# weidafeng/Efficient-SlowFast

Hardware: AMD Instinct MI355X
Metric: clips/sec (8x8 224^2 SlowFast-R50+CMDA, train step fwd+bwd+allreduce+SGD) (higher is better)
Workload: dtype f32

## Files before the change

efficient-slowfast_amd/sfhip/__init__.py:

```python
import ctypes
import os

import torch

_HERE = os.path.dirname(os.path.abspath(__file__))
_LIB_PATH = os.environ.get("SF_LIB") or os.path.join(_HERE, "libsfhip.so")
_lib = None

ACT_NONE, ACT_RELU, ACT_SIGMOID, ACT_SOFTMAX, ACT_HSIGMOID, ACT_RELU6 = 0, 1, 2, 3, 4, 5


def _act(relu):
    return ACT_RELU6 if relu == 6 else (ACT_RELU if relu else ACT_NONE)
SF_EINVAL, SF_EALIGN, SF_ELAUNCH, SF_ENOTTAKEN = -1, -2, -3, -4
_ERR = {-1: "SF_EINVAL (inconsistent descriptor)", -2: "SF_EALIGN", -3: "SF_ELAUNCH (hip launch failed)",
        -4: "SF_ENOTTAKEN (shape not served by this specialised entry point)"}
_REFUSED = (SF_EALIGN, SF_ENOTTAKEN)


class SfhipError(RuntimeError):
    pass


class ConvDesc(ctypes.Structure):
# ... 80 lines not shown
    "sf_attn_fwd_ws_floats": (_cl, [_ci] * 3),
    "sf_attn_products_per_fp32": (_ci, [_ci]),
    "sf_attn_fwd_ws": (_ci, _ATTN_FWD + [_vp, _vp]),
    "sf_attn_bwd": (_ci, [_vp, _ci] * 4 + [_vp, _vp, _vp] + [_vp, _ci] * 3 + [_ci] * 4 + [_vp]),
    "sf_attn_bwd_fused_ws_floats": (_cl, [_ci] * 3),
    "sf_attn_bwd_fused": (_ci, [_vp, _ci] * 4 + [_vp, _vp, _vp] + [_vp, _ci] * 3 + [_ci] * 3 + [_vp, _vp]),
    "sf_attn_bwd_variant": (_ci, [_ci] * 3),
    "sf_attn_tune": (_ci, [_ci, _ci]),
    "sf_xattn_accepts": (_ci, [_cl, _cl, _ci, _ci]),
    "sf_xattn_bwd_ws_floats": (_cl, [_ci, _cl, _cl, _ci, _ci]),
    "sf_xattn_fwd": (_ci, [_vp, _ci] * 4 + [_vp, _ci, _cl, _cl, _ci, _ci, _cf, _vp]),
    "sf_xattn_bwd": (_ci, [_vp, _ci] * 4 + [_vp, _vp] + [_vp, _ci] * 3 + [_ci, _ci, _cl, _cl, _ci, _ci, _cf, _vp, _vp]),
    "sf_assoc_accepts": (_ci, [_cl, _cl, _ci, _ci]),
    "sf_gram_splits": (_ci, [_ci, _cl, _ci, _ci]),
    "sf_gram_ws_floats": (_cl, [_ci, _cl, _ci, _ci]),
    "sf_gram": (_ci, [_vp, _ci, _vp, _ci, _vp, _vp, _ci, _cl, _ci, _ci, _cf, _vp, _vp]),
    "sf_rowmat": (_ci, [_vp, _ci, _vp, _vp, _ci, _ci, _cl, _ci, _ci, _cf, _ci, _vp]),
    "sf_channel_stats_ws_floats": (_cl, [_ci]),
    "sf_channel_stats": (_ci, _VIEW + [_cl, _ci, _vp, _vp, _vp, _vp]),
    "sf_bn_train_stats": (_ci, _VIEW + [_cl, _ci, _vp, _vp, _cf, _cf] + [_vp] * 9),
    "sf_bn_train_stats_split": (_ci, _VIEW + [_ci, _cl, _ci, _ci, _vp, _vp, _cf, _cf] + [_vp] * 9),
    "sf_bn_train_stats_merge": (_ci, [_vp, _ci, _ci, _vp, _vp, _cf, _cf] + [_vp] * 8),
    "sf_affine_fwd": (_ci, _VIEW + [_ci] * 5 + [_vp, _vp] + _VIEW + [_ci, _ci] + _VIEW + [_ci, _vp]),
    "sf_affine_fwd_split": (_ci, _VIEW + [_ci] * 6 + [_vp, _vp] + _VIEW + [_ci, _ci] + _VIEW + [_ci, _vp]),
    "sf_affine_fwd_mask": (_ci, _VIEW + [_ci] * 5 + [_vp, _vp] + _VIEW + [_ci] + _VIEW + [_vp, _vp]),
    "sf_bn_bwd_ws_floats": (_cl, [_ci]),
    "sf_bn_bwd_reduce": (_ci, _BN_BWD + [_vp]),
    "sf_bn_bwd_reduce_acc": (_ci, _BN_BWD + [_vp, _vp, _vp]),
    "sf_bn_bwd_reduce_split": (_ci, _BN_BWD_SPLIT + [_vp]),
    "sf_bn_bwd_apply": (_ci, _BN_BWD + _BN_APPLY_TAIL),
    "sf_bn_bwd_apply_first": (_ci, _BN_BWD + _BN_APPLY_TAIL),
    "sf_bn_bwd_apply_split": (_ci, _BN_BWD_SPLIT + _BN_APPLY_TAIL),
    "sf_bn_frozen_bwd": (_ci, _VIEW * 3 + [_ci] * 7 + [_vp] * 3 + _VIEW * 2 + [_ci] + [_vp] * 4),
    "sf_head_act_mean": (_ci, [_vp, _ci, _ci, _ci, _ci, _vp, _vp]),
    "sf_head_act_mean_bwd": (_ci, [_vp, _vp, _ci, _ci, _ci, _ci, _vp, _ci, _vp]),
    "sf_copy_channels": (_ci, _VIEW * 2 + [_ci, _cl, _ci, _vp]),
    "sf_channel_shuffle": (_ci, _VIEW * 2 + [_ci, _cl, _ci, _ci, _vp]),
    "sf_gather_add": (_ci, _VIEW + [_ci] + _VIEW + [_cl, _ci, _ci, _vp]),
    "sf_bcast_add": (_ci, _VIEW + [_ci, _cl, _ci, _vp, _cf, _vp]),
    "sf_rowdot": (_ci, _VIEW * 2 + [_cl, _ci, _cf, _vp, _vp]),
    "sf_axpy": (_ci, _VIEW + [_cf] + _VIEW + [_cl, _ci, _ci, _vp]),
    "sf_act_bwd": (_ci, _VIEW * 2 + [_ci] + _VIEW + [_cl, _ci, _ci, _vp]),
    "sf_sigmoid_bwd": (_ci, [_vp, _vp, _vp, _cl, _ci, _vp]),
    "sf_row_softmax_fwd": (_ci, _VIEW + [_cl, _ci, _cf, _vp]),
    "sf_row_softmax_bwd": (_ci, _VIEW * 2 + [_cl, _ci, _cf, _vp]),
    "sf_roi_tpool_fwd": (_ci, _VIEW + [_ci] * 5 + [_vp, _vp]),
    "sf_roi_align_max_fwd": (_ci, [_vp] + [_ci] * 4 + [_vp, _ci, _ci, _cf, _ci] + _VIEW + [_vp, _vp]),
    "sf_roi_align_max_bwd": (_ci, _VIEW + [_vp, _vp] + [_ci] * 7 + [_cf, _ci] + _VIEW + [_ci, _vp]),
    "sf_epilogue_bwd": (_ci, _VIEW * 2 + [_ci] * 6 + [_vp, _ci] + _VIEW + [_ci] + _VIEW + [_ci, _vp]),
    "sf_epilogue_bwd_act": (_ci, _VIEW * 2 + [_ci] * 6 + [_vp, _ci, _ci] + _VIEW + [_ci] + _VIEW + [_ci, _vp]),
    "sf_cam_weights": (_ci, _VIEW + [_ci] * 5 + [_vp, _vp]),
    "sf_cam_map_ws_floats": (_cl, [_ci] * 4),
    "sf_cam_map": (_ci, _VIEW + [_vp] + [_ci] * 5 + [_vp, _vp, _vp, _vp]),
    "sf_ctx_pool_parts": (_ci, [_cl]),
    "sf_ctx_pool_ws_floats": (_cl, [_ci, _cl, _ci]),
    "sf_ctx_pool_fwd": (_ci, _VIEW + [_ci, _cl, _ci] + [_vp] * 6),
    "sf_ctx_pool_bwd": (_ci, _VIEW + [_ci, _cl, _ci] + [_vp] * 5 + _VIEW + [_ci, _vp, _vp, _ci, _vp, _vp]),
    "sf_sample_affine_ws_floats": (_cl, [_ci, _cl, _ci]),
    "sf_sample_affine_fwd": (_ci, _VIEW + [_ci, _cl, _ci, _vp, _vp] + _VIEW + [_vp]),
    "sf_sample_affine_bwd": (_ci, _VIEW * 2 + [_ci, _cl, _ci, _vp] + _VIEW + [_ci, _vp, _vp, _vp, _vp]),
    "sf_stripe_pool_fwd": (_ci, _VIEW + [_ci] * 7 + _VIEW + [_vp, _vp]),
    "sf_stripe_add_fwd": (_ci, _VIEW * 2 + [_ci] * 6 + _VIEW + [_vp]),
    "sf_stripe_pool_bwd": (_ci, _VIEW * 3 + [_vp] + [_ci] * 6 + _VIEW + [_ci, _vp]),
}
EXPORTS = list(_SIGNATURES)

# ... 811 lines not shown
    _call("sf_conv_fwd_grouped", ctypes.byref(d), groups, 0, dz.ptr(), _ptr(wtp), None, None,
          out.ptr() if accumulate else None, out.ptr(), tag=("conv", dz.rows, taps * (dz.C // groups), cin),
          what="sf_conv_fwd_grouped(transposed)")
    return out


def conv_wgrad_grouped(x, dz, groups, kernel, stride=(1, 1, 1), padding=(0, 0, 0), dilation=(1, 1, 1),
                       cin_pad=None, finish_into=None):
    _require_gpu(x.buf, "conv_wgrad_grouped")
    cin_g, cout = x.C // groups, dz.C
    assert x.C % groups == 0 and cout % groups == 0
    cin_pad = _pad16(cin_g) if cin_pad is None else cin_pad
    kT, kH, kW = kernel
    d = _conv_desc(x, (dz.T, dz.H, dz.W), 0, 0, cout, kernel, stride, padding, dilation, cin_pad=cin_pad)
    S = lib().sf_conv_wgrad_grouped_splits(ctypes.byref(d), groups)
    if S <= 0:
        raise SfhipError("sf_conv_wgrad_grouped_splits: %d -> %d channels in %d groups" % (x.C, cout, groups))
    part = torch.empty((S, cout, kT * kH * kW, cin_pad), dtype=torch.float32, device=x.buf.device)
    _call("sf_conv_wgrad_grouped", ctypes.byref(d), groups, x.ptr(), dz.ptr(), dz.cs, dz.coff, _ptr(part),
          tag=("conv", dz.rows, kT * kH * kW * cin_g, cout))
    if finish_into is not None:
        dst = finish_into
        assert dst.is_contiguous() and dst.dtype == torch.float32 and dst.numel() == cout * cin_g * kT * kH * kW
        _call("sf_conv_wgrad_finish", _ptr(part), S, cout, kT * kH * kW, cin_pad, cin_g, 0, _ptr(dst), 1)
        return None
    return part.sum(0) if S > 1 else part[0]


def unpack_conv_weight_grad(dwp, shape):
    cout, cin, kT, kH, kW = shape
    return dwp[:, :, :cin].permute(0, 2, 1).reshape(cout, cin, kT, kH, kW).contiguous()


def bn_bwd(dy, y, z, mean, invstd, gamma, relu, rep=1, dres=None, dz_out=None, dgamma_out=None, nsplit=1,
           sync=None, grad_sink=None, mask=None, dres_overwrite=False):
    C = z.C
    dev = z.buf.device
    mean, invstd, gamma = mean.contiguous(), invstd.contiguous(), gamma.detach().contiguous()
    dbeta = torch.empty((nsplit * C,), dtype=torch.float32, device=dev)
    dgamma = torch.empty((nsplit * C,), dtype=torch.float32, device=dev)
    ws = torch.empty((lib().sf_bn_bwd_ws_floats(C),), dtype=torch.float32, device=dev)
    yp, ycs, yco = (y.ptr(), y.cs, y.coff) if y is not None else (None, 0, 0)
    code = 2 if relu == 6 else (1 if relu else 0)
    if mask is not None and relu:
        assert rep == 1 and nsplit == 1 and mask.numel() == z.rows * (C // 4)
        yp, ycs, yco, code = _ptr(mask), C // 4, 0, 3
    head = (dy.ptr(), dy.cs, dy.coff, yp, ycs, yco, z.ptr(), z.cs, z.coff, z.N, z.T, z.H, z.W, C)
    tail = (rep, code, _ptr(mean), _ptr(invstd))
    split = (nsplit,) if nsplit > 1 else ()
    reduce_fn = "sf_bn_bwd_reduce_split" if nsplit > 1 else "sf_bn_bwd_reduce"
    apply_fn = "sf_bn_bwd_apply_split" if nsplit > 1 else "sf_bn_bwd_apply"
    if dres_overwrite:
        assert dres is not None and nsplit == 1
        apply_fn = "sf_bn_bwd_apply_first"
    if grad_sink is not None:
        assert nsplit == 1 and dgamma_out is None
        _call("sf_bn_bwd_reduce_acc", *head, *tail, _ptr(dbeta), _ptr(dgamma), _ptr(ws), _ptr(grad_sink[1]),
              _ptr(grad_sink[0]))
    else:
        _call(reduce_fn, *head, *split, *tail, _ptr(dbeta), _ptr(dgamma), _ptr(ws))
    db_apply, dg_apply = (dbeta, dgamma) if sync is None else sync(dbeta, dgamma)
    out = z if dz_out is None else dz_out
    _call(apply_fn, *head, *split, *tail, _ptr(gamma), _ptr(db_apply), _ptr(dg_apply), out.ptr(), out.cs, out.coff,
          dres.ptr() if dres is not None else None, dres.cs if dres is not None else 0,
          dres.coff if dres is not None else 0)
    if dgamma_out is not None:
        if nsplit > 1:
            dgamma_out[0][:C] = dgamma.view(nsplit, C).sum(0)
            dgamma_out[1][:C] = dbeta.view(nsplit, C).sum(0)
        else:
            dgamma_out[0][:C] = dgamma
            dgamma_out[1][:C] = dbeta
    return out, dgamma, dbeta


def bn_frozen_bwd(dy, y, z, mean, invstd, gamma, relu, rep=1, dres=None, dres_overwrite=False, dz_out=None,
                  grads=None, mask=None):
    if dy is None or z is None or (relu and mask is None and y is None):
        raise SfhipError("bn_frozen_bwd: dy, z and (with an activation) y or its mask are required")
    for name, a in (("dy", dy), ("z", z), ("dz", dz_out), ("dres", dres), ("y", y if (relu and mask is None) else None)):
        if a is not None:
            _require_gpu(a.buf, "bn_frozen_bwd(%s)" % name)
    C, dev = z.C, z.buf.device
    if dres is not None and rep != 1:
        raise SfhipError("bn_frozen_bwd: the residual's gradient is only defined without a T repeat (rep = %d)" % rep)
    if (dy.N, dy.T, dy.H, dy.W, dy.C) != (z.N, z.T * rep, z.H, z.W, C):
        raise SfhipError("bn_frozen_bwd: dy %r does not match z %r repeated %d times" % (dy, z, rep))
    vecs = [("mean", mean), ("invstd", invstd)] + ([("gamma", gamma)] if gamma is not None else [])
    for name, v in vecs:
        _require_gpu(v, "bn_frozen_bwd(%s)" % name)
        if v.numel() < C or not v.is_contiguous():
            raise SfhipError("bn_frozen_bwd: %s must be a contiguous tensor of at least %d floats" % (name, C))
    dgp = dbp = ws = None
    if grads is not None:
        for name, v in (("dgamma", grads[0]), ("dbeta", grads[1])):
            _require_gpu(v, "bn_frozen_bwd(%s)" % name)
            if v.numel() < C or not v.is_contiguous():
                raise SfhipError("bn_frozen_bwd: %s must be a contiguous tensor of at least %d floats" % (name, C))
# ... 556 lines not shown
```

efficient-slowfast_amd/slowfast/models/engine.py:

```python
import os
import threading
import weakref

import torch
import torch.nn as nn

import sfhip
from sfhip import Act

_tls = threading.local()


class internal(object):

    def __enter__(self):
        self.prev = getattr(_tls, "depth", 0)
        _tls.depth = self.prev + 1

    def __exit__(self, *a):
        _tls.depth = self.prev


def is_internal():
    return getattr(_tls, "depth", 0) > 0
# ... 263 lines not shown
        _tls.pending_side = None
    else:
        _tls.pending_side = side
    if t is not None:
        t.record(bwd_fork)
    return [out0, out1]


def join_pending(device):
    pend = getattr(_tls, "pending_side", None)
    if pend is not None:
        _sync_streams(pend, torch.cuda.current_stream(device))
        _tls.pending_side = None


class taping(object):
    def __init__(self, t):
        self.t = t

    def __enter__(self):
        self.prev = getattr(_tls, "tape", None)
        _tls.tape = self.t

    def __exit__(self, *a):
        _tls.tape = self.prev


def _colsum(act):
    mean, _ = sfhip.channel_stats(act)
    return mean * float(act.rows)


def _record_conv(x, conv_weight, conv_bias, wp_shape, gsrc, kernel, stride, padding, dilation, x_needs_grad=True,
                 cin=None, unpack=None, fold_kw=0):
    t = tape()
    if t is None:
        return
    cout = conv_weight.shape[0]

    def wgrad(g):
        tgt = t.pgrad_target(conv_weight)
        if tgt is not None:
            real_cin = conv_weight.shape[1]
            sfhip.conv_wgrad(x, g, cout, kernel, stride, padding, dilation, cin=cin, cin_pad=wp_shape[2],
                             finish_into=(tgt, real_cin, fold_kw))
        else:
            dwp = sfhip.conv_wgrad(x, g, cout, kernel, stride, padding, dilation, cin=cin, cin_pad=wp_shape[2])
            t.add_pgrad(conv_weight, unpack(dwp) if unpack else sfhip.unpack_conv_weight_grad(dwp, conv_weight.shape))
        if conv_bias is not None:
            t.add_pgrad(conv_bias, _colsum(g))

    def bwd():
        g = gsrc() if callable(gsrc) else gsrc
        dev = x.buf.device
        if not t.param_grads:
            pass
        elif OVERLAP_PATHS and not t.capturing and not t.serial and x_needs_grad and dev.type == "cuda":
            cur = torch.cuda.current_stream(dev)
            wg = _companion_stream(cur)
            _sync_streams(cur, wg)
            with torch.cuda.stream(wg):
                wgrad(g)
            g.buf.record_stream(wg)
            x.buf.record_stream(wg)
            t.joins.add(wg)
        else:
            wgrad(g)
        if x_needs_grad:
            if conv_weight.dim() == 5 and tuple(conv_weight.shape[2:]) == tuple(kernel):
                wtp = _packed_pair(conv_weight)[1]
            else:
                wtp = _cached_t(conv_weight, "_sf_wtp", _key(conv_weight),
                                lambda: sfhip.pack_conv_weight(conv_weight.detach().reshape(
                                    conv_weight.shape[0], conv_weight.shape[1], *kernel).transpose(0, 1).contiguous()))
            fresh = t.grad_of_uninitialised(x)
            if fresh is not None:
                sfhip.conv_dgrad(g, wtp, x, kernel, stride, padding, dilation, out=fresh, accumulate=False)
            else:
                sfhip.conv_dgrad(g, wtp, x, kernel, stride, padding, dilation, out=t.grad_of(x), accumulate=True)

    t.record(bwd)


_PCACHE = {}


_CAPTURE_KEEP = {}


def _keep_if_capturing(obj):
    if getattr(_tls, "capturing", False):
        _CAPTURE_KEEP[id(obj)] = obj
    return obj


def _cached_t(tensor, slot, key, make):
    store = tensor.__dict__.setdefault("_sf_cache", {})
    c = store.get(slot)
    if c is None or c[0] != key:
        with torch.no_grad():
            c = (key, make())
        store[slot] = c
    return _keep_if_capturing(c[1])


_PARAM_EPOCH = 0


def parameters_changed(*_unused):
    global _PARAM_EPOCH
    _PARAM_EPOCH += 1


def replay(graph):
# ... 77 lines not shown
        vec = group_gather_sum(torch.cat([lm, lvar.double() + lm * lm]), nd, ng) / nd
        mean64, meansqr = vec[:z.C], vec[z.C:]
        var64 = (meansqr - mean64 * mean64).clamp_min(0.0)
        mean, var = mean64.float(), var64.float()
        invstd = torch.rsqrt(var64 + bn.eps).float()
        scale = (bn.weight.detach() * invstd).contiguous()
        shift = (bn.bias.detach() - mean * scale).contiguous()
        if track:
            bn.running_mean += m * (mean - bn.running_mean)
            bn.running_var += m * (var - bn.running_var)
            bn.__dict__.pop("_sf_affine", None)

        def sync(dbeta, dgamma):
            tot = group_gather_sum(torch.cat([dbeta, dgamma]).double(), nd, ng) / nd
            return tot[:dbeta.numel()].float().contiguous(), tot[dbeta.numel():].float().contiguous()

        return mean, invstd, scale, shift, 1, bn.weight, sync
    if conv_stats is not None:
        mean, invstd, scale, shift = sfhip.bn_train_stats_merge(
            conv_stats, z.C, bn.weight, bn.bias, bn.eps, m, bn.running_mean if track else None,
            bn.running_var if track else None)
    else:
        mean, invstd, scale, shift = sfhip.bn_train_stats(
            z, bn.weight, bn.bias, bn.eps, m, bn.running_mean if track else None, bn.running_var if track else None)
    if track:
        bn.__dict__.pop("_sf_affine", None)
        _bump(bn.num_batches_tracked)
    return mean, invstd, scale, shift, 1, bn.weight, None


def bn_train_apply(bn, z, res=None, relu=False, rep=1, out=None, out_reserve=(0, 0), keep=None, out_cmul=1,
                   conv_stats=None):
    check_bn(bn)
    with torch.no_grad():
        mean, invstd, scale, shift, nsplit, gamma_b, sync = _bn_train_stats(bn, z, conv_stats)
    zz = z if keep is None else z.slice(0, keep)
    nk = z.C if keep is None else keep
    if keep is not None:
        assert nsplit == 1, "channel-sliced BN (GhostModule) is only defined for plain BatchNorm3d"
        scale, shift = scale[:keep].contiguous(), shift[:keep].contiguous()
    t = tape()
    shuffled = t is not None and out_cmul != 1
    mk = {} if (t is not None and relu) else None
    if shuffled:
        y = sfhip.affine(zz, scale.contiguous(), shift.contiguous(), res=res, relu=relu, rep=rep, nsplit=nsplit,
                         mask=mk)
    else:
        y = sfhip.affine(zz, scale.contiguous(), shift.contiguous(), res=res, relu=relu, rep=rep, out=out,
                         out_reserve=out_reserve, out_cmul=out_cmul, nsplit=nsplit, mask=mk)
    mask = mk.get("bytes") if mk else None
    if t is not None:
        if _GRAD_SINK:
            dg = db = None
        else:
            dg = torch.zeros(z.C, dtype=torch.float32, device=z.buf.device)
            db = torch.zeros(z.C, dtype=torch.float32, device=z.buf.device)
        sel = slice(None) if nsplit > 1 else slice(0, nk)

        def bwd():
            dres, first = None, False
            if res is not None:
                fresh = t.grad_of_uninitialised(res) if (nsplit == 1 and res.C == zz.C and rep == 1) else None
                dres, first = (fresh, True) if fresh is not None else (t.grad_of(res), False)
            wt = t.pgrad_target(bn.weight) if (nsplit == 1 and getattr(bn, "weight", None) is not None) else None
            bt = t.pgrad_target(bn.bias) if wt is not None else None
            if wt is not None and bt is not None:
                sfhip.bn_bwd(t.grad_of(y), y, zz, mean[sel], invstd[sel], gamma_b[sel], relu, rep=rep, dres=dres,
                             dz_out=zz, sync=sync, grad_sink=(wt, bt), mask=mask, dres_overwrite=first)
            else:
                dg_ = dg if dg is not None else torch.zeros(z.C, dtype=torch.float32, device=z.buf.device)
                db_ = db if db is not None else torch.zeros(z.C, dtype=torch.float32, device=z.buf.device)
                sfhip.bn_bwd(t.grad_of(y), y, zz, mean[sel], invstd[sel], gamma_b[sel], relu, rep=rep, dres=dres,
                             dz_out=zz, dgamma_out=(dg_, db_), nsplit=nsplit, sync=sync, mask=mask,
                             dres_overwrite=first)
            if keep is not None and keep < z.C:
                rest = z.slice(keep, z.C - keep)
                sfhip.axpy(rest, rest, alpha=0.0, accumulate=False)
            if (wt is None or bt is None) and getattr(bn, "weight", None) is not None:
                t.add_pgrad(bn.weight, dg_)
                t.add_pgrad(bn.bias, db_)

        t.record(bwd)
    if shuffled:
        return copy_channels(y, out, out_cmul=out_cmul)
    return y


def bn_affine(bn, conv_bias=None):
    check_bn(bn)
    stat = bn.bn if _sub_bn(bn) else bn
    w = getattr(bn, "weight", None)
    b = getattr(bn, "bias", None)

    def make():
        inv = 1.0 / torch.sqrt(stat.running_var + stat.eps)
        scale = w * inv if w is not None else inv
        bias = -stat.running_mean * scale
        if b is not None:
            bias = bias + b
        if conv_bias is not None:
            bias = bias + scale * conv_bias
        return scale.detach().contiguous(), bias.detach().contiguous()

    return _cached(bn, "_sf_affine", _key(w, b, stat.running_mean, stat.running_var, conv_bias), make)


def _taped_training():
# ... 194 lines not shown
    if t is not None:
        t.record(lambda: sfhip.channel_shuffle(t.grad_of(out), t.grad_of(x), x.C // groups, accumulate=True))
    return out


def _is_grouped(conv):
    return 1 < conv.groups and not (conv.groups == conv.in_channels and conv.out_channels == conv.in_channels)


def conv_bn_act(x, conv, bn=None, relu=False, res=None, out=None, out_reserve=(0, 0), out_cmul=1, cout=None,
                shuffle=False):
    if _is_grouped(conv):
        assert out_cmul == 1 and cout is None, "grouped convs have their own shuffle"
        if bn is not None and bn_unfused(bn):
            z = grouped_conv(x, conv, bias=conv.bias)
            _record_grouped_conv(x, conv, z)
            if not shuffle:
                return bn_apply(bn, z, res=res, relu=relu, out=out, out_reserve=out_reserve)
            y = bn_apply(bn, z, res=res, relu=relu)
            return channel_shuffle(y, conv.groups, out=out, out_reserve=out_reserve)
        scale, bias = bn_affine(bn, conv.bias) if bn is not None else (None, conv.bias)
        t = tape()
        if t is not None and not isinstance(t, EvalTape):
            raise NotImplementedError("taped grouped conv without a norm layer behind it")
        y = grouped_conv(x, conv, scale=scale, bias=bias, relu=relu, res=res, out=out, out_reserve=out_reserve,
                         shuffle=shuffle)
        if t is not None:
            _record_eval_grouped_conv(t, x, conv, y, scale, relu, res, shuffle)
        return y
    assert not shuffle or conv.groups == 1, "channel_shuffle of a depthwise conv's output is not used by any model"
    wp = packed_weight(conv)
    if bn is not None and bn_unfused(bn):
        k, s, p, d = conv.kernel_size, conv.stride, conv.padding, conv.dilation
        st = None
        if conv.groups == 1:
            want = bn.training and _plain_bn(bn) and bn.affine
            z = sfhip.conv(x, wp, k, s, p, d, bias=conv.bias, stats=want)
            z, st = z if want else (z, None)
            _record_conv(x, conv.weight, conv.bias, wp.shape, z, k, s, p, d)
        else:
            ones = _cached(conv, "_sf_ones", (conv.out_channels, str(x.buf.device)),
                           lambda: torch.ones(conv.out_channels, dtype=torch.float32, device=x.buf.device))
            z = sfhip.dwconv(x, wp, k, s, p, scale=ones if conv.bias is not None else None, bias=conv.bias)
            t = tape()
            if t is not None:
                def bwd_dw():
                    tgt = t.pgrad_target(conv.weight)
                    wpk = packed_weight(conv)
                    if tgt is not None:
                        sfhip.dwconv_bwd(x, z, wpk, k, s, p, dx=t.grad_of(x), into=tgt)
                    else:
                        dw = sfhip.dwconv_bwd(x, z, wpk, k, s, p, dx=t.grad_of(x))
                        t.add_pgrad(conv.weight, dw[:, :x.C].t().contiguous())
                    if conv.bias is not None:
                        t.add_pgrad(conv.bias, _colsum(z))

                t.record(bwd_dw)
        return bn_apply(bn, z, res=res, relu=relu, out=out, out_reserve=out_reserve, keep=cout, out_cmul=out_cmul,
                        conv_stats=st)
    if bn is not None:
        scale, bias = bn_affine(bn, conv.bias)
    else:
        scale, bias = None, conv.bias
    k, s, p, d = conv.kernel_size, conv.stride, conv.padding, conv.dilation
    if conv.groups == 1:
        y = sfhip.conv(x, wp, k, s, p, d, scale=scale, bias=bias, relu=relu, res=res, out=out,
                       out_reserve=out_reserve, out_cmul=out_cmul)
        t = tape()
        if isinstance(t, EvalTape):
            _record_eval_conv(t, x, conv, wp, y, scale, relu, res, out_cmul)
        elif t is not None:
            if (res is not None and relu) or out_cmul != 1:
                raise NotImplementedError("taped conv without a norm layer but with a residual behind an activation "
                                          "or an interleaved store")
            if res is not None:
                def bwd_res():
                    sfhip.axpy(t.grad_of(y), t.grad_of(res), 1.0, accumulate=True)
                t.record(bwd_res)
            if relu:
                def masked():
                    dz = sfhip.new_act(y, y.N, y.T, y.H, y.W, y.C)
                    return sfhip.act_bwd(t.grad_of(y), y, relu, dz, accumulate=False)
                _record_conv(x, conv.weight, conv.bias, wp.shape, masked, k, s, p, d)
            else:
                _record_conv(x, conv.weight, conv.bias, wp.shape, lambda: t.grad_of(y), k, s, p, d)
        return y
    assert d == (1, 1, 1)
    if scale is None and bias is not None:
        scale = torch.ones_like(bias)
    y = sfhip.dwconv(x, wp, k, s, p, scale=scale, bias=bias, relu=relu, res=res, out=out, cout=cout,
                     out_cmul=out_cmul)
    t = tape()
# ... 371 lines not shown
```

include/sfhip.h:

```cpp
#ifndef SFHIP_H
#define SFHIP_H
#ifdef __cplusplus
extern "C" {
#endif

#define SF_OK 0
#define SF_EINVAL (-1)
#define SF_EALIGN (-2)
#define SF_ELAUNCH (-3)
#define SF_ENOTTAKEN (-4)

#define SF_ACT_NONE 0
#define SF_ACT_RELU 1
#define SF_ACT_SIGMOID 2
#define SF_ACT_SOFTMAX 3
#define SF_ACT_HSIGMOID 4
#define SF_ACT_RELU6 5

int sf_abi_version(void);
const char* sf_build_arch(void);

int sf_ncthw_to_ndhwc(const float* src, float* dst, int N, int C, int T, int H, int W,
                      int cpad, int ph, int pw, int Wp, void* stream);
int sf_ndhwc_to_ncthw(const float* src, int cs, int coff, float* dst, int N, int C, int T, int H,
// ... 136 lines not shown
int sf_conv_wgrad_grouped(const sf_conv_desc* d, int groups, const float* x, const float* dz, int dz_cs, int dz_coff,
                          float* partial, void* stream);
int sf_conv_wgrad_finish(const float* partial, int S, int Cout, int packed_taps, int cin_pad, int Cin, int fold_kw,
                         float* dst, int accumulate, void* stream);

#define SF_BN_MASK_BYTES 3
long sf_bn_bwd_ws_floats(int C);
int sf_affine_fwd_mask(const float* x, int cs, int coff, int N, int T, int H, int W, int C, const float* scale,
                       const float* bias, const float* res, int res_cs, int res_coff, int act, float* out,
                       int out_cs, int out_coff, unsigned char* mask, void* stream);
int sf_bn_bwd_reduce(const float* dy, int dy_cs, int dy_coff, const float* y, int y_cs, int y_coff,
                     const float* z, int z_cs, int z_coff, int N, int T, int H, int W, int C, int rep, int relu,
                     const float* mean, const float* invstd, float* dbeta, float* dgamma, float* ws, void* stream);
int sf_bn_bwd_reduce_acc(const float* dy, int dy_cs, int dy_coff, const float* y, int y_cs, int y_coff,
                         const float* z, int z_cs, int z_coff, int N, int T, int H, int W, int C, int rep, int relu,
                         const float* mean, const float* invstd, float* dbeta, float* dgamma, float* ws,
                         float* dbeta_acc, float* dgamma_acc, void* stream);
int sf_bn_bwd_apply(const float* dy, int dy_cs, int dy_coff, const float* y, int y_cs, int y_coff,
                    const float* z, int z_cs, int z_coff, int N, int T, int H, int W, int C, int rep, int relu,
                    const float* mean, const float* invstd, const float* gamma, const float* dbeta,
                    const float* dgamma, float* dz, int dz_cs, int dz_coff, float* dres, int dres_cs,
                    int dres_coff, void* stream);
int sf_bn_bwd_apply_first(const float* dy, int dy_cs, int dy_coff, const float* y, int y_cs, int y_coff,
                          const float* z, int z_cs, int z_coff, int N, int T, int H, int W, int C, int rep, int relu,
                          const float* mean, const float* invstd, const float* gamma, const float* dbeta,
                          const float* dgamma, float* dz, int dz_cs, int dz_coff, float* dres, int dres_cs,
                          int dres_coff, void* stream);
int sf_bn_frozen_bwd(const float* dy, int dy_cs, int dy_coff, const float* y, int y_cs, int y_coff,
                     const float* z, int z_cs, int z_coff, int N, int T, int H, int W, int C, int rep, int relu,
                     const float* mean, const float* invstd, const float* gamma, float* dz, int dz_cs, int dz_coff,
                     float* dres, int dres_cs, int dres_coff, int dres_accumulate, float* dbeta, float* dgamma,
                     float* ws, void* stream);

int sf_maxpool_bwd(const sf_pool_desc* d, const float* x, const float* y, const float* dy, int dy_cs,
                   int dy_coff, float* dx, int dx_cs, int dx_coff, void* stream);
int sf_maxpool_bwd_first(const sf_pool_desc* d, const float* x, const float* y, const float* dy, int dy_cs,
                         int dy_coff, float* dx, int dx_cs, int dx_coff, void* stream);

int sf_tmax_dot(const float* x, int cs, int coff, int N, int T, int H, int W, int C, int alpha, const float* dz,
                int dz_cs, int dz_coff, float* out, float* ws, void* stream);
int sf_eca_bwd_apply(const float* x, int cs, int coff, int N, int T, int H, int W, int C, int alpha,
                     const float* dz, int dz_cs, int dz_coff, const float* gate, const float* dpool, float* dx,
                     int dx_cs, int dx_coff, void* stream);

int sf_eca_gate_bwd(const float* dg, const float* pooled, const float* w3, int N, int C, float dpool_scale,
                    float* gate, float* dpool, float* dw3, void* stream);

int sf_dwconv_dgrad(const sf_conv_desc* d, const float* dz, int dz_cs, int dz_coff, const float* w_packed,
                    float* dx, int dx_cs, int dx_coff, int C, void* stream);
long sf_dwconv_wgrad_ws_floats(const sf_conv_desc* d, int C);
int sf_dwconv_wgrad(const sf_conv_desc* d, const float* x, const float* dz, int dz_cs, int dz_coff, int C,
                    float* dw, float* ws, void* stream);
int sf_dwconv_wgrad_param(const sf_conv_desc* d, const float* x, const float* dz, int dz_cs, int dz_coff, int C,
                          float* dw_param, int accumulate, float* ws, void* stream);
int sf_gather_add(const float* in, int in_cs, int in_coff, int in_cmul, float* out, int out_cs, int out_coff,
                  long rows, int C, int accumulate, void* stream);

int sf_bcast_add(float* g, int cs, int coff, int N, long rows_per_n, int C, const float* v, float scale,
                 void* stream);
int sf_rowdot(const float* a, int a_cs, int a_coff, const float* b, int b_cs, int b_coff, long rows, int C,
              float scale, float* out, void* stream);
int sf_axpy(const float* a, int a_cs, int a_coff, float alpha, float* out, int out_cs, int out_coff, long rows,
            int C, int accumulate, void* stream);
int sf_bn_train_stats_split(const float* x, int cs, int coff, int N, long rows_per_sample, int C, int nsplit,
                            const float* gamma, const float* beta, float eps, float momentum, float* run_mean,
                            float* run_var, float* mean, float* var, float* invstd, float* scale, float* shift,
// ... 108 lines not shown
```

Before: 153.8.

## Fuse BN backward apply with pointwise conv dgrad and wgrad for narrow inputs

Adds a HIP kernel that computes the BN backward apply (masked ReLU, normalisation terms) for a tile of rows, keeps the resulting dz in LDS, and immediately feeds it to MFMA-based 1x1 conv dgrad and per-block wgrad partials. The engine defers the conv backward closure and routes eligible pointwise conv+BN layers (Cin<64, Cout<=256) through this fused path, falling back when the kernel refuses. This is meant to remove writing dz to global memory and re-reading it in separate dgrad and wgrad kernels, plus their launches. In exchange it adds a large LDS footprint per block, a new partial-sum reduction step, and more complex tape ordering.

Result: no change. 153.4, median of 2 (-0.3%).

```diff
diff --git a/efficient-slowfast_amd/csrc/conv_pw_bnbwd.hip b/efficient-slowfast_amd/csrc/conv_pw_bnbwd.hip
--- /dev/null
+++ b/efficient-slowfast_amd/csrc/conv_pw_bnbwd.hip
@@ -0,0 +1,298 @@
+#include "common.h"
+
+namespace {
+
+constexpr int PB_TR = 64;
+constexpr int PB_NT = 256;
+
+struct PwBnArgs {
+  const float* dy; int dy_cs, dy_coff;
+  const unsigned char* mask;
+  const float* z; int z_cs, z_coff;
+  const float *mean, *invstd, *gamma, *dbeta, *dgamma;
+  float inv_m;
+  const float* x; int x_cs, x_coff;
+  const float* wt; int cout_pad;
+  float* dx; int dx_cs, dx_coff, dx_acc;
+  float* dres; int dres_cs, dres_coff, dres_acc;
+  float* part; int cin_pad;
+  long rows;
+  int Cin, Cout;
+};
+
+__host__ __device__ inline int pb_lds_floats(int Cin, int Cout) {
+  const int cout16 = (Cout + 15) / 16 * 16, cin16 = (Cin + 15) / 16 * 16;
+  return 5 * cout16 + cin16 * (cout16 + 4) + PB_TR * (cout16 + 4) + PB_TR * (cin16 + 4);
+}
+
+template <int CPW, int NCI>
+__global__ __launch_bounds__(PB_NT) void conv_pw_bn_bwd_kernel(const PwBnArgs a) {
+  extern __shared__ float lds[];
+  const int tid = threadIdx.x, lane = tid & 63, wave = tid >> 6;
+  const int li = lane & 15, lq = lane >> 4;
+  const int C = a.Cout, Cin = a.Cin;
+  const unsigned cv = (unsigned)C >> 2, xv = (unsigned)Cin >> 2;
+  const int nco = (C + 15) >> 4, nci = (Cin + 15) >> 4;
+  const int cout16 = nco * 16, WS = cout16 + 4, XS = nci * 16 + 4;
+  float* const c_mu = lds;
+  float* const c_is = c_mu + cout16;
+  float* const c_k0 = c_is + cout16;
+  float* const c_db = c_k0 + cout16;
+  float* const c_dg = c_db + cout16;
+  float* const wl = c_dg + cout16;
+  float* const dzs = wl + nci * 16 * WS;
+  float* const xs = dzs + PB_TR * WS;
+
+  for (int c = tid; c < cout16; c += PB_NT) {
+    const bool ok = c < C;
+    const float is = ok ? a.invstd[c] : 0.f;
+    c_mu[c] = ok ? a.mean[c] : 0.f;
+    c_is[c] = is;
+    c_k0[c] = ok ? a.gamma[c] * is : 0.f;
+    c_db[c] = ok ? a.dbeta[c] * a.inv_m : 0.f;
+    c_dg[c] = ok ? a.dgamma[c] : 0.f;
+  }
+  {
+    const int wv = WS >> 2;
+    for (int i = tid; i < nci * 16 * wv; i += PB_NT) {
+      const int ci = i / wv, c = (i - ci * wv) * 4;
+      f32x4 v = {0.f, 0.f, 0.f, 0.f};
+      if (ci < Cin && c < C) {
+        v = *reinterpret_cast<const f32x4*>(a.wt + (long)ci * a.cout_pad + c);
+      }
+      *reinterpret_cast<f32x4*>(wl + ci * WS + c) = v;
+    }
+    for (int i = tid; i < PB_TR * wv; i += PB_NT) *reinterpret_cast<f32x4*>(dzs + i * 4) = (f32x4){0.f, 0.f, 0.f, 0.f};
+    for (int i = tid; i < PB_TR * (XS >> 2); i += PB_NT)
+      *reinterpret_cast<f32x4*>(xs + i * 4) = (f32x4){0.f, 0.f, 0.f, 0.f};
+  }
+  __syncthreads();
+
+  f32x4 wacc[CPW][NCI];
+#pragma unroll
+  for (int p = 0; p < CPW; ++p)
+#pragma unroll
+    for (int ct = 0; ct < NCI; ++ct) wacc[p][ct] = (f32x4){0.f, 0.f, 0.f, 0.f};
+
+  const long tiles = (a.rows + PB_TR - 1) / PB_TR;
+  const long t0 = tiles * blockIdx.x / gridDim.x, t1 = tiles * (blockIdx.x + 1) / gridDim.x;
+  const int cv_shift = (cv & (cv - 1u)) == 0u ? __builtin_ctz(cv) : -1;
+  const int xv_shift = (xv & (xv - 1u)) == 0u ? __builtin_ctz(xv) : -1;
+  const unsigned nvec = PB_TR * cv, nxv = PB_TR * xv;
+
+  for (long t = t0; t < t1; ++t) {
+    const long r0 = t * PB_TR;
+    const unsigned nr = (unsigned)((a.rows - r0) < PB_TR ? (a.rows - r0) : PB_TR);
+    f32x4 xr[4];
+#pragma unroll
+    for (int u = 0; u < 4; ++u) {
+      const unsigned idx = (unsigned)tid + (unsigned)u * PB_NT;
+      const unsigned row = xv_shift >= 0 ? idx >> xv_shift : idx / xv;
+      const unsigned c = (idx - row * xv) * 4u;
+      xr[u] = (f32x4){0.f, 0.f, 0.f, 0.f};
+      if (idx < nxv && row < nr) xr[u] = *reinterpret_cast<const f32x4*>(a.x + (r0 + row) * a.x_cs + a.x_coff + c);
+    }
+    for (unsigned base = 0; base < nvec; base += 4u * PB_NT) {
+      f32x4 gv[4], zq[4], rv[4];
+      unsigned mb[4];
+#pragma unroll
+      for (int u = 0; u < 4; ++u) {
+        const unsigned idx = base + (unsigned)u * PB_NT + (unsigned)tid;
+        const unsigned row = cv_shift >= 0 ? idx >> cv_shift : idx / cv;
+        const unsigned c4 = idx - row * cv;
+        gv[u] = zq[u] = rv[u] = (f32x4){0.f, 0.f, 0.f, 0.f};
+        mb[u] = 0xFu;
+        if (idx < nvec && row < nr) {
+          const long r = r0 + row;
+          gv[u] = *reinterpret_cast<const f32x4*>(a.dy + r * a.dy_cs + a.dy_coff + c4 * 4u);
+          zq[u] = *reinterpret_cast<const f32x4*>(a.z + r * a.z_cs + a.z_coff + c4 * 4u);
+          if (a.mask) mb[u] = a.mask[r * cv + c4];
+          if (a.dres && a.dres_acc) rv[u] = *reinterpret_cast<const f32x4*>(a.dres + r * a.dres_cs + a.dres_coff + c4 * 4u);
+        }
+      }
+      if (base == 0) {
+#pragma unroll
+        for (int u = 0; u < 4; ++u) {
+          const unsigned idx = (unsigned)tid + (unsigned)u * PB_NT;
+          const unsigned row = xv_shift >= 0 ? idx >> xv_shift : idx / xv;
+          const unsigned c = (idx - row * xv) * 4u;
+          if (idx < nxv) *reinterpret_cast<f32x4*>(xs + row * XS + c) = xr[u];
+        }
+      }
+#pragma unroll
+      for (int u = 0; u < 4; ++u) {
+        const unsigned idx = base + (unsigned)u * PB_NT + (unsigned)tid;
+        const unsigned row = cv_shift >= 0 ? idx >> cv_shift : idx / cv;
+        const unsigned c4 = idx - row * cv;
+        if (idx < nvec) {
+          const int c = (int)c4 * 4;
+          const f32x4 is = *reinterpret_cast<const f32x4*>(c_is + c), mu = *reinterpret_cast<const f32x4*>(c_mu + c);
+          const f32x4 k0 = *reinterpret_cast<const f32x4*>(c_k0 + c), db = *reinterpret_cast<const f32x4*>(c_db + c);
+          const f32x4 dg = *reinterpret_cast<const f32x4*>(c_dg + c);
+          f32x4 ov, gg;
+#pragma unroll
+          for (int e = 0; e < 4; ++e) {
+            gg[e] = ((mb[u] >> e) & 1u) ? gv[u][e] : 0.f;
+            const float xh = (zq[u][e] - mu[e]) * is[e];
+            ov[e] = k0[e] * (gg[e] - db[e] - xh * dg[e] * a.inv_m);
+          }
+          const bool valid = row < nr;
+          if (!valid) ov = (f32x4){0.f, 0.f, 0.f, 0.f};
+          *reinterpret_cast<f32x4*>(dzs + row * WS + c) = ov;
+          if (valid && a.dres)
+            *reinterpret_cast<f32x4*>(a.dres + (r0 + row) * a.dres_cs + a.dres_coff + c) = rv[u] + gg;
+        }
+      }
+    }
+    __syncthreads();
+    {
+      const unsigned row_l = 16u * (unsigned)wave + (unsigned)li;
+      const bool rvalid = row_l < nr;
+      float* const dxp = a.dx + (r0 + row_l) * a.dx_cs + a.dx_coff + 4 * lq;
+      f32x4 dacc[NCI], prior[NCI];
+#pragma unroll
+      for (int ct = 0; ct < NCI; ++ct) {
+        dacc[ct] = prior[ct] = (f32x4){0.f, 0.f, 0.f, 0.f};
+        if (a.dx_acc && rvalid && 16 * ct + 4 * lq < Cin) prior[ct] = *reinterpret_cast<const f32x4*>(dxp + 16 * ct);
+      }
+      const float* const bsrc = dzs + row_l * WS + 4 * lq;
+      const float* const asrc = wl + li * WS + 4 * lq;
+      for (int kk = 0; kk < nco; ++kk) {
+        const f32x4 b = *reinterpret_cast<const f32x4*>(bsrc + 16 * kk);
+#pragma unroll
+        for (int ct = 0; ct < NCI; ++ct) {
+          if (ct < nci) {
+            const f32x4 aw = *reinterpret_cast<const f32x4*>(asrc + 16 * ct * WS + 16 * kk);
+#pragma unroll
+            for (int s = 0; s < 4; ++s) dacc[ct] = __builtin_amdgcn_mfma_f32_16x16x4f32(aw[s], b[s], dacc[ct], 0, 0, 0);
+          }
+        }
+      }
+#pragma unroll
+      for (int ct = 0; ct < NCI; ++ct)
+        if (rvalid && 16 * ct + 4 * lq < Cin) *reinterpret_cast<f32x4*>(dxp + 16 * ct) = prior[ct] + dacc[ct];
+    }
+    {
+      const int kend = ((int)nr + 3) & ~3;
+      for (int k0 = 0; k0 < kend; k0 += 4) {
+        const int row = k0 + lq;
+        float av[NCI];
+#pragma unroll
+        for (int ct = 0; ct < NCI; ++ct) av[ct] = ct < nci ? xs[row * XS + 16 * ct + li] : 0.f;
+#pragma unroll
+        for (int p = 0; p < CPW; ++p) {
+          const int cot = wave + 4 * p;
+          if (cot < nco) {
+            const float b = dzs[row * WS + 16 * cot + li];
+#pragma unroll
+            for (int ct = 0; ct < NCI; ++ct)
+              if (ct < nci) wacc[p][ct] = __builtin_amdgcn_mfma_f32_16x16x4f32(av[ct], b, wacc[p][ct], 0, 0, 0);
+          }
+        }
+      }
+    }
+    __syncthreads();
+  }
+  float* const pp = a.part + (long)blockIdx.x * C * a.cin_pad;
+#pragma unroll
+  for (int p = 0; p < CPW; ++p) {
+    const int co = 16 * (wave + 4 * p) + li;
+    if (co < C) {
+#pragma unroll
+      for (int ct = 0; ct < NCI; ++ct)
+        if (ct < nci) *reinterpret_cast<f32x4*>(pp + (long)co * a.cin_pad + 16 * ct + 4 * lq) = wacc[p][ct];
+    }
+  }
+}
+
+bool pb_shape_ok(long rows, int Cin, int Cout) {
+  return rows > 0 && Cin >= 4 && Cout >= 4 && Cin <= 64 && Cout <= 256 && (Cin % 4) == 0 && (Cout % 4) == 0;
+}
+
+template <int CPW, int NCI>
+int pb_launch(const PwBnArgs& a, int S, int lds_bytes, hipStream_t stream) {
+  static SfLdsAttr attr;
+  if (lds_bytes > 65536 &&
+      !sf_ensure_dyn_lds(attr, reinterpret_cast<const void*>(&conv_pw_bn_bwd_kernel<CPW, NCI>), lds_bytes))
+    return SF_ELAUNCH;
+  hipLaunchKernelGGL((conv_pw_bn_bwd_kernel<CPW, NCI>), dim3(S), dim3(PB_NT), (size_t)lds_bytes, stream, a);
+  SF_CHECK_LAUNCH();
+  return SF_OK;
+}
+
+}
+
+extern "C" int sf_conv_pw_bn_bwd_parts(long rows, int Cin, int Cout) {
+  if (!pb_shape_ok(rows, Cin, Cout)) return 0;
+  const long tiles = (rows + PB_TR - 1) / PB_TR;
+  const int cin_pad = (Cin + 15) / 16 * 16;
+  const int per_cu = (160 * 1024) / (pb_lds_floats(Cin, Cout) * 4);
+  const long cap = 256L * (per_cu < 1 ? 1 : (per_cu > 4 ? 4 : per_cu));
+  long s = rows / (2L * cin_pad);
+  if (s > cap) s = cap;
+  if (s > tiles) s = tiles;
+  if (s < 1) s = 1;
+  return (int)s;
+}
+
+extern "C" int sf_conv_pw_bn_bwd(const sf_conv_desc* d, const float* dy, int dy_cs, int dy_coff, const float* y,
+                                 int y_cs, int y_coff, const float* z, int z_cs, int z_coff, int nsplit, int rep,
+                                 int relu, const float* mean, const float* invstd, const float* gamma,
+                                 const float* dbeta, const float* dgamma, float inv_m, const float* x,
+                                 const float* wt, int cout_pad, float* dx, int dx_cs, int dx_coff,
+                                 int dx_accumulate, float* dres, int dres_cs, int dres_coff, int dres_accumulate,
+                                 float* partial, void* stream) {
+  if (!d || !dy || !z || !mean || !invstd || !gamma || !dbeta || !dgamma || !x || !wt || !dx || !partial)
+    return SF_EINVAL;
+  if (d->N <= 0 || d->Ti <= 0 || d->Hi <= 0 || d->Wi <= 0 || d->To <= 0 || d->Ho <= 0 || d->Wo <= 0 || d->Cin <= 0 ||
+      d->Cout <= 0 || nsplit <= 0 || rep <= 0 || relu < 0 || relu > 3 || (relu && !y))
+    return SF_EINVAL;
+  const int Cin = d->Cin, Cout = d->Cout;
+  if (d->in_cs < d->in_coff + Cin || dy_cs < dy_coff + Cout || z_cs < z_coff + Cout || dx_cs < dx_coff + Cin ||
+      (dres && dres_cs < dres_coff + Cout) || dy_coff < 0 || z_coff < 0 || dx_coff < 0 || d->in_coff < 0 ||
+      (dres && dres_coff < 0) || cout_pad < Cout)
+    return SF_EINVAL;
+  if (d->kT != 1 || d->kH != 1 || d->kW != 1 || d->sT != 1 || d->sH != 1 || d->sW != 1 || d->pT != 0 || d->pH != 0 ||
+      d->pW != 0 || d->dT != 1 || d->dH != 1 || d->dW != 1 || d->transposed || d->out_cmul != 1)
+    return SF_ENOTTAKEN;
+  if (d->To != d->Ti || d->Ho != d->Hi || d->Wo != d->Wi) return SF_ENOTTAKEN;
+  const long rows = (long)d->N * d->To * d->Ho * d->Wo;
+  if (!pb_shape_ok(rows, Cin, Cout) || nsplit != 1 || rep != 1 || (relu != 0 && relu != 3)) return SF_ENOTTAKEN;
+  if (d->cin_pad != (Cin + 15) / 16 * 16 || (cout_pad % 4) != 0) return SF_ENOTTAKEN;
+  if (relu == 3 && (y_cs != Cout / 4 || y_coff != 0)) return SF_EINVAL;
+  if ((dy_cs | dy_coff | z_cs | z_coff | dx_cs | dx_coff | d->in_cs | d->in_coff) % 4 != 0 ||
+      (dres && ((dres_cs | dres_coff) % 4) != 0) || !sf_aligned16(dy) || !sf_aligned16(z) || !sf_aligned16(x) ||
+      !sf_aligned16(dx) || !sf_aligned16(wt) || !sf_aligned16(partial) || (dres && !sf_aligned16(dres)))
+    return SF_ENOTTAKEN;
+  const int S = sf_conv_pw_bn_bwd_parts(rows, Cin, Cout);
+  if (S <= 0) return SF_ENOTTAKEN;
+  PwBnArgs a;
+  a.dy = dy; a.dy_cs = dy_cs; a.dy_coff = dy_coff;
+  a.mask = relu == 3 ? reinterpret_cast<const unsigned char*>(y) : nullptr;
+  a.z = z; a.z_cs = z_cs; a.z_coff = z_coff;
+  a.mean = mean; a.invstd = invstd; a.gamma = gamma; a.dbeta = dbeta; a.dgamma = dgamma;
+  a.inv_m = inv_m > 0.f ? inv_m : 1.f / (float)rows;
+  a.x = x; a.x_cs = d->in_cs; a.x_coff = d->in_coff;
+  a.wt = wt; a.cout_pad = cout_pad;
+  a.dx = dx; a.dx_cs = dx_cs; a.dx_coff = dx_coff; a.dx_acc = dx_accumulate ? 1 : 0;
+  a.dres = dres; a.dres_cs = dres_cs; a.dres_coff = dres_coff; a.dres_acc = dres_accumulate ? 1 : 0;
+  a.part = partial; a.cin_pad = d->cin_pad;
+  a.rows = rows; a.Cin = Cin; a.Cout = Cout;
+  const int lds_bytes = pb_lds_floats(Cin, Cout) * 4;
+  const int nco = (Cout + 15) / 16, nci = (Cin + 15) / 16;
+  const int cpw = (nco + 3) / 4;
+  hipStream_t s = (hipStream_t)stream;
+  if (cpw <= 1) {
+    if (nci <= 1) return pb_launch<1, 1>(a, S, lds_bytes, s);
+    if (nci <= 2) return pb_launch<1, 2>(a, S, lds_bytes, s);
+    return pb_launch<1, 4>(a, S, lds_bytes, s);
+  }
+  if (cpw <= 2) {
+    if (nci <= 1) return pb_launch<2, 1>(a, S, lds_bytes, s);
+    if (nci <= 2) return pb_launch<2, 2>(a, S, lds_bytes, s);
+    return pb_launch<2, 4>(a, S, lds_bytes, s);
+  }
+  if (nci <= 1) return pb_launch<4, 1>(a, S, lds_bytes, s);
+  if (nci <= 2) return pb_launch<4, 2>(a, S, lds_bytes, s);
+  return pb_launch<4, 4>(a, S, lds_bytes, s);
+}
diff --git a/efficient-slowfast_amd/sfhip/__init__.py b/efficient-slowfast_amd/sfhip/__init__.py
--- a/efficient-slowfast_amd/sfhip/__init__.py
+++ b/efficient-slowfast_amd/sfhip/__init__.py
@@ -136,6 +136,9 @@
     "sf_bn_bwd_apply_first": (_ci, _BN_BWD + _BN_APPLY_TAIL),
     "sf_bn_bwd_apply_split": (_ci, _BN_BWD_SPLIT + _BN_APPLY_TAIL),
     "sf_bn_frozen_bwd": (_ci, _VIEW * 3 + [_ci] * 7 + [_vp] * 3 + _VIEW * 2 + [_ci] + [_vp] * 4),
+    "sf_conv_pw_bn_bwd_parts": (_ci, [_cl, _ci, _ci]),
+    "sf_conv_pw_bn_bwd": (_ci, [_CD] + _VIEW * 3 + [_ci] * 3 + [_vp] * 5 + [_cf, _vp, _vp, _ci] + (_VIEW + [_ci]) * 2 +
+                          [_vp, _vp]),
     "sf_head_act_mean": (_ci, [_vp, _ci, _ci, _ci, _ci, _vp, _vp]),
     "sf_head_act_mean_bwd": (_ci, [_vp, _vp, _ci, _ci, _ci, _ci, _vp, _ci, _vp]),
     "sf_copy_channels": (_ci, _VIEW * 2 + [_ci, _cl, _ci, _vp]),
@@ -1013,8 +1016,36 @@
     return dwp[:, :, :cin].permute(0, 2, 1).reshape(cout, cin, kT, kH, kW).contiguous()
 
 
+ROUTES = {"pw_bn_bwd": 0, "pw_bn_bwd_refused": 0}
+
+
+def conv_pw_bn_bwd(conv, bn_head, nsplit, bn_tail, gamma, dbeta, dgamma, dres, dres_overwrite):
+    x, wtp, cin_pad, kernel, stride, padding, dilation, dx, dx_acc = conv
+    N, T, H, W, cout = bn_head[9:14]
+    S = lib().sf_conv_pw_bn_bwd_parts(N * T * H * W, x.C, cout)
+    if S <= 0 or wtp.dim() != 3 or wtp.shape[1] != 1:
+        ROUTES["pw_bn_bwd_refused"] += 1
+        return None
+    d = _conv_desc(x, (T, H, W), 0, 0, cout, kernel, stride, padding, dilation, cin_pad=cin_pad)
+    part = torch.empty((S, cout, 1, cin_pad), dtype=torch.float32, device=x.buf.device)
+    rep, code, mean, invstd = bn_tail
+    rc = _call("sf_conv_pw_bn_bwd", ctypes.byref(d), *bn_head[:9], nsplit, rep, code, mean, invstd, _ptr(gamma),
+               _ptr(dbeta), _ptr(dgamma), 0.0, x.ptr(), _ptr(wtp), wtp.shape[2], dx.ptr(), dx.cs, dx.coff,
+               1 if dx_acc else 0, dres.ptr() if dres is not None else None, dres.cs if dres is not None else 0,
+               dres.coff if dres is not None else 0, 0 if dres_overwrite else 1, _ptr(part), allow=_REFUSED)
+    ROUTES["pw_bn_bwd" if rc == 0 else "pw_bn_bwd_refused"] += 1
+    return part if rc == 0 else None
+
+
+def conv_wgrad_finish(part, cin, dst, accumulate=True):
+    S, cout, taps, cin_pad = part.shape
+    assert dst.is_contiguous() and dst.dtype == torch.float32 and dst.numel() == cout * cin * taps, (dst.shape, part.shape)
+    _call("sf_conv_wgrad_finish", _ptr(part), S, cout, taps, cin_pad, cin, 0, _ptr(dst), 1 if accumulate else 0)
+    return dst
+
+
 def bn_bwd(dy, y, z, mean, invstd, gamma, relu, rep=1, dres=None, dz_out=None, dgamma_out=None, nsplit=1,
-           sync=None, grad_sink=None, mask=None, dres_overwrite=False):
+           sync=None, grad_sink=None, mask=None, dres_overwrite=False, fuse_conv=None):
     C = z.C
     dev = z.buf.device
     mean, invstd, gamma = mean.contiguous(), invstd.contiguous(), gamma.detach().contiguous()
@@ -1042,9 +1073,16 @@
         _call(reduce_fn, *head, *split, *tail, _ptr(dbeta), _ptr(dgamma), _ptr(ws))
     db_apply, dg_apply = (dbeta, dgamma) if sync is None else sync(dbeta, dgamma)
     out = z if dz_out is None else dz_out
-    _call(apply_fn, *head, *split, *tail, _ptr(gamma), _ptr(db_apply), _ptr(dg_apply), out.ptr(), out.cs, out.coff,
-          dres.ptr() if dres is not None else None, dres.cs if dres is not None else 0,
-          dres.coff if dres is not None else 0)
+    part = None
+    if fuse_conv is not None:
+        part = conv_pw_bn_bwd(fuse_conv[:-1], head, nsplit, tail, gamma, db_apply, dg_apply, dres, dres_overwrite)
+    if part is not None:
+        fuse_conv[-1].append(part)
+        out = None
+    else:
+        _call(apply_fn, *head, *split, *tail, _ptr(gamma), _ptr(db_apply), _ptr(dg_apply), out.ptr(), out.cs,
+              out.coff, dres.ptr() if dres is not None else None, dres.cs if dres is not None else 0,
+              dres.coff if dres is not None else 0)
     if dgamma_out is not None:
         if nsplit > 1:
             dgamma_out[0][:C] = dgamma.view(nsplit, C).sum(0)
diff --git a/efficient-slowfast_amd/slowfast/models/engine.py b/efficient-slowfast_amd/slowfast/models/engine.py
--- a/efficient-slowfast_amd/slowfast/models/engine.py
+++ b/efficient-slowfast_amd/slowfast/models/engine.py
@@ -319,10 +319,10 @@
 
 
 def _record_conv(x, conv_weight, conv_bias, wp_shape, gsrc, kernel, stride, padding, dilation, x_needs_grad=True,
-                 cin=None, unpack=None, fold_kw=0):
+                 cin=None, unpack=None, fold_kw=0, defer=False):
     t = tape()
     if t is None:
-        return
+        return None
     cout = conv_weight.shape[0]
 
     def wgrad(g):
@@ -337,7 +337,7 @@
         if conv_bias is not None:
             t.add_pgrad(conv_bias, _colsum(g))
 
-    def bwd():
+    def bwd(dx_to=None):
         g = gsrc() if callable(gsrc) else gsrc
         dev = x.buf.device
         if not t.param_grads:
@@ -360,13 +360,28 @@
                 wtp = _cached_t(conv_weight, "_sf_wtp", _key(conv_weight),
                                 lambda: sfhip.pack_conv_weight(conv_weight.detach().reshape(
                                     conv_weight.shape[0], conv_weight.shape[1], *kernel).transpose(0, 1).contiguous()))
-            fresh = t.grad_of_uninitialised(x)
+            if dx_to is not None:
+                fresh = None if dx_to[1] else dx_to[0]
+            else:
+                fresh = t.grad_of_uninitialised(x)
             if fresh is not None:
                 sfhip.conv_dgrad(g, wtp, x, kernel, stride, padding, dilation, out=fresh, accumulate=False)
             else:
                 sfhip.conv_dgrad(g, wtp, x, kernel, stride, padding, dilation, out=t.grad_of(x), accumulate=True)
 
+    if defer:
+        return bwd
     t.record(bwd)
+    return None
+
+
+def _pw_bn_fusable(t, x, conv, bn):
+    one, zero = (1, 1, 1), (0, 0, 0)
+    return (t is not None and t.param_grads and not isinstance(t, EvalTape) and x.buf.is_cuda and conv.groups == 1
+            and conv.bias is None and tuple(conv.kernel_size) == one and tuple(conv.stride) == one
+            and tuple(conv.padding) == zero and tuple(conv.dilation) == one and bn.training and _plain_bn(bn)
+            and bn.affine and conv.in_channels < 64 and conv.out_channels <= 256 and conv.in_channels % 4 == 0
+            and conv.out_channels % 4 == 0 and x.C == conv.in_channels)
 
 
 _PCACHE = {}
@@ -510,6 +525,7 @@
 def bn_train_apply(bn, z, res=None, relu=False, rep=1, out=None, out_reserve=(0, 0), keep=None, out_cmul=1,
                    conv_stats=None):
     check_bn(bn)
+    fuse_conv, _tls.pw_fuse = getattr(_tls, "pw_fuse", None), None
     with torch.no_grad():
         mean, invstd, scale, shift, nsplit, gamma_b, sync = _bn_train_stats(bn, z, conv_stats)
     zz = z if keep is None else z.slice(0, keep)
@@ -542,15 +558,32 @@
                 dres, first = (fresh, True) if fresh is not None else (t.grad_of(res), False)
             wt = t.pgrad_target(bn.weight) if (nsplit == 1 and getattr(bn, "weight", None) is not None) else None
             bt = t.pgrad_target(bn.bias) if wt is not None else None
+            fc, dx_to, parts = None, None, []
+            if fuse_conv is not None and nsplit == 1 and rep == 1 and keep is None and sync is None and \
+                    (not relu or mask is not None):
+                cx, cw = fuse_conv[0], fuse_conv[1]
+                fresh = t.grad_of_uninitialised(cx)
+                dx_to = (fresh, False) if fresh is not None else (t.grad_of(cx), True)
+                fc = (cx, _packed_pair(cw)[1]) + tuple(fuse_conv[2:7]) + dx_to + (parts,)
             if wt is not None and bt is not None:
                 sfhip.bn_bwd(t.grad_of(y), y, zz, mean[sel], invstd[sel], gamma_b[sel], relu, rep=rep, dres=dres,
-                             dz_out=zz, sync=sync, grad_sink=(wt, bt), mask=mask, dres_overwrite=first)
+                             dz_out=zz, sync=sync, grad_sink=(wt, bt), mask=mask, dres_overwrite=first, fuse_conv=fc)
             else:
                 dg_ = dg if dg is not None else torch.zeros(z.C, dtype=torch.float32, device=z.buf.device)
                 db_ = db if db is not None else torch.zeros(z.C, dtype=torch.float32, device=z.buf.device)
                 sfhip.bn_bwd(t.grad_of(y), y, zz, mean[sel], invstd[sel], gamma_b[sel], relu, rep=rep, dres=dres,
                              dz_out=zz, dgamma_out=(dg_, db_), nsplit=nsplit, sync=sync, mask=mask,
-                             dres_overwrite=first)
+                             dres_overwrite=first, fuse_conv=fc)
+            if parts:
+                cw = fuse_conv[1]
+                tgt = t.pgrad_target(cw)
+                if tgt is not None:
+                    sfhip.conv_wgrad_finish(parts[0], cw.shape[1], tgt, accumulate=True)
+                else:
+                    t.add_pgrad(cw, sfhip.conv_wgrad_finish(parts[0], cw.shape[1], torch.empty_like(cw),
+                                                            accumulate=False))
+            elif fuse_conv is not None:
+                fuse_conv[7](dx_to)
             if keep is not None and keep < z.C:
                 rest = z.slice(keep, z.C - keep)
                 sfhip.axpy(rest, rest, alpha=0.0, accumulate=False)
@@ -811,12 +844,16 @@
     wp = packed_weight(conv)
     if bn is not None and bn_unfused(bn):
         k, s, p, d = conv.kernel_size, conv.stride, conv.padding, conv.dilation
-        st = None
+        st, fc = None, None
         if conv.groups == 1:
             want = bn.training and _plain_bn(bn) and bn.affine
             z = sfhip.conv(x, wp, k, s, p, d, bias=conv.bias, stats=want)
             z, st = z if want else (z, None)
-            _record_conv(x, conv.weight, conv.bias, wp.shape, z, k, s, p, d)
+            if _pw_bn_fusable(tape(), x, conv, bn) and cout is None:
+                fc = (x, conv.weight, wp.shape[2], k, s, p, d,
+                      _record_conv(x, conv.weight, conv.bias, wp.shape, z, k, s, p, d, defer=True))
+            else:
+                _record_conv(x, conv.weight, conv.bias, wp.shape, z, k, s, p, d)
         else:
             ones = _cached(conv, "_sf_ones", (conv.out_channels, str(x.buf.device)),
                            lambda: torch.ones(conv.out_channels, dtype=torch.float32, device=x.buf.device))
@@ -835,8 +872,12 @@
                         t.add_pgrad(conv.bias, _colsum(z))
 
                 t.record(bwd_dw)
-        return bn_apply(bn, z, res=res, relu=relu, out=out, out_reserve=out_reserve, keep=cout, out_cmul=out_cmul,
-                        conv_stats=st)
+        _tls.pw_fuse = fc
+        try:
+            return bn_apply(bn, z, res=res, relu=relu, out=out, out_reserve=out_reserve, keep=cout,
+                            out_cmul=out_cmul, conv_stats=st)
+        finally:
+            _tls.pw_fuse = None
     if bn is not None:
         scale, bias = bn_affine(bn, conv.bias)
     else:
diff --git a/include/sfhip.h b/include/sfhip.h
--- a/include/sfhip.h
+++ b/include/sfhip.h
@@ -192,6 +192,14 @@
                      float* dres, int dres_cs, int dres_coff, int dres_accumulate, float* dbeta, float* dgamma,
                      float* ws, void* stream);
 
+int sf_conv_pw_bn_bwd_parts(long rows, int Cin, int Cout);
+int sf_conv_pw_bn_bwd(const sf_conv_desc* d, const float* dy, int dy_cs, int dy_coff, const float* y, int y_cs,
+                      int y_coff, const float* z, int z_cs, int z_coff, int nsplit, int rep, int relu,
+                      const float* mean, const float* invstd, const float* gamma, const float* dbeta,
+                      const float* dgamma, float inv_m, const float* x, const float* wt, int cout_pad, float* dx,
+                      int dx_cs, int dx_coff, int dx_accumulate, float* dres, int dres_cs, int dres_coff,
+                      int dres_accumulate, float* partial, void* stream);
+
 int sf_maxpool_bwd(const sf_pool_desc* d, const float* x, const float* y, const float* dy, int dy_cs,
                    int dy_coff, float* dx, int dx_cs, int dx_coff, void* stream);
 int sf_maxpool_bwd_first(const sf_pool_desc* d, const float* x, const float* y, const float* dy, int dy_cs,
```
